# IvanIZ/BenchPush

Measured on AMD Instinct MI355X. Metric: env-steps/sec at N=4096 envs (ship-ice-v0), 1/2/4/8 MI355X, higher is better.
Workload: dtype f64

## Files before the change

benchpush_amd/csrc/bp_capi.hip:

```cpp
#include <hip/hip_runtime.h>

#include <cstdio>
#include <cstdlib>
#include <algorithm>
#include <cstring>
#include <map>
#include <mutex>
#include <string>
#include <vector>

#include <fcntl.h>
#include <sys/file.h>
#include <sys/stat.h>
#include <unistd.h>

#include "bp_host_bd.hpp"
#include "bp_boxdelivery.hpp"
#include "bp_policy.hpp"
#include "bp_render.hpp"
#include "bp_state.hpp"
#include "bp_swath.hpp"
#include "bp_lattice.hpp"
#include "bp_track.hpp"
#include "bp_rrt.hpp"
// ... 52 lines not shown
    std::vector<int> bd_map_of_trial;
    bool timing = false;
    std::vector<hipEvent_t> ev;
    size_t ev_used = 0;
    unsigned long long *cost_ring = nullptr;
    int cost_n = 0;
    int *r_order = nullptr;
    unsigned *r_rgb = nullptr;
    bp_render_prim *r_prims = nullptr;
    int r_nunder = 0, r_nover = 0;
    bool r_table = false;
    unsigned long long scen_hash = 0xCBF29CE484222325ull;
    BpStateLayout st_layout;
    BpStateSeg *st_table = nullptr;
    unsigned long long st_layout_id = 0;
};
#define BP_COST_RING 1024

static int fail(bp_handle *h, int code, const std::string &msg)
{
    if (h) h->err = msg;
    return code;
}
#define HIPCHK(h, call)                                                                                       \
    do {                                                                                                      \
        hipError_t _e = (call);                                                                               \
        if (_e != hipSuccess) return fail((h), BP_EHIP, std::string(#call) + ": " + hipGetErrorString(_e));    \
    } while (0)

struct DevGuard {
    int prev = -1;
// ... 496 lines not shown
    const bool box = h->P.env_kind == BP_ENV_BOX;
    const int cells = box ? h->B.SH * h->B.SW : 0;
    h->st_layout = bp_state_layout(h->D, h->Q, h->nbcap, box, cells);
    const BpStateLayout &L = h->st_layout;
    if (L.nseg >= BP_STATE_MAXSEG || (L.bytes >> 4) >= 0xFFFFFFFFull) return fail(h, BP_EINVAL, "state record layout out of range");
    unsigned long long id = bp_state_structure_id(L, h->P.env_kind, box ? h->bdcfg.task : 0, h->nbcap, cells);
    if (box) id = bp_fnv1a(&h->bdcfg, sizeof(h->bdcfg), id);
    else id = bp_fnv1a(&h->cfg, sizeof(h->cfg), id);
    h->st_layout_id = bp_fnv1a_i64((long long)h->scen_hash, id);
    int rc = dalloc(h, &h->st_table, (size_t)BP_STATE_MAXSEG);
    if (rc) return rc;
    HIPCHK(h, hipMemcpy(h->st_table, L.seg, sizeof(BpStateSeg) * L.nseg, hipMemcpyHostToDevice));
    return BP_OK;
}

static int kind_of(int ctype, int group, int btype) { return ctype | (group << 8) | (btype << 16); }

int bp_load_scenarios(bp_handle *h, int32_t T, int32_t F, int32_t V, const double *verts, const int32_t *counts,
                      const double *centres, const double *starts, const int32_t *nfloes)
{
    if (!h || T <= 0 || F < 0 || V <= 0 || !starts || !nfloes) return BP_EINVAL;
    if (h->loaded) return fail(h, BP_ESTATE, "scenarios already loaded");
    if (h->P.env_kind != BP_ENV_SHIP_ICE) return fail(h, BP_ESTATE, "handle was created for another environment");
    BP_DEVICE(h);
    using namespace bpgeom;
    std::vector<std::vector<Shape>> trials(T);
    for (int t = 0; t < T; t++) {
        std::vector<Shape> &bodies = trials[t];
        Shape ship;
        build_ship(h->cfg.ship_verts, h->cfg.num_ship_verts, starts[3 * t], starts[3 * t + 1], starts[3 * t + 2], ship);
// ... 2 lines not shown
        bodies.push_back(ship);
        if (nfloes[t] > F) return fail(h, BP_EINVAL, "nfloes > F");
        for (int f = 0; f < nfloes[t]; f++) {
            const int n = counts[(size_t)t * F + f];
            if (n < 3) continue;
            if (n > V) return fail(h, BP_EINVAL, "vertex count > V");
            Shape s;
            if (!build_floe(verts + ((size_t)t * F + f) * V * 2, n, centres[((size_t)t * F + f) * 2],
                            centres[((size_t)t * F + f) * 2 + 1], h->cfg.density, h->cfg.poly_radius, s))
                continue;
            s.radius = h->cfg.poly_radius; s.e = h->cfg.elasticity; s.u = h->cfg.friction;
            s.kind = kind_of(2, 0, BODY_DYNAMIC);
            bodies.push_back(s);
        }
    }
    const int rc_up = upload_trials(h, trials);
    return rc_up ? rc_up : state_setup(h);
}

int bp_load_maze(bp_handle *h, int32_t T, int32_t nbox, const double *centres, int32_t nwalls, const double *walls, const double *start)
{
    if (!h || T <= 0 || nbox < 0 || nwalls < 0 || nwalls > 16 || !walls || !start || (nbox > 0 && !centres)) return BP_EINVAL;
    if (h->loaded) return fail(h, BP_ESTATE, "scenarios already loaded");
    if (h->P.env_kind != BP_ENV_MAZE) return fail(h, BP_ESTATE, "handle was created for another environment");
    BP_DEVICE(h);
    using namespace bpgeom;
    const bp_config &cf = h->cfg;
    std::vector<std::vector<Shape>> trials(T);
    for (int t = 0; t < T; t++) {
        std::vector<Shape> &bodies = trials[t];
        for (int k = 0; k <= cf.num_wheels; k++) {
            Shape s;
// ... 34 lines not shown
    {
        std::vector<double> packed(norm.size());
        for (size_t i = 0; i < norm.size(); i++) packed[i] = wall[i] ? -norm[i] : norm[i];
        double *d_pk;
        if ((rc = dalloc(h, &d_pk, packed.size()))) return rc;
        HIPCHK(h, hipMemcpy(d_pk, packed.data(), sizeof(double) * packed.size(), hipMemcpyHostToDevice));
        h->D.maze_obs_map = d_pk;
    }
    double *d_raw;
    if ((rc = dalloc(h, &d_raw, h->goal_raw.size()))) return rc;
    HIPCHK(h, hipMemcpy(d_raw, h->goal_raw.data(), sizeof(double) * h->goal_raw.size(), hipMemcpyHostToDevice));
    h->D.goal_raw = d_raw;
    h->scen_hash = bp_fnv1a(wall.data(), wall.size(), h->scen_hash);
    h->scen_hash = bp_fnv1a(norm.data(), sizeof(double) * norm.size(), h->scen_hash);
    h->scen_hash = bp_fnv1a(h->goal_raw.data(), sizeof(double) * h->goal_raw.size(), h->scen_hash);
    const int rc_up = upload_trials(h, trials);
    return rc_up ? rc_up : state_setup(h);
}

int bp_get_goal_map(bp_handle *h, double *out_host, int32_t *grid_h, int32_t *grid_w)
{
    if (!h) return BP_EINVAL;
    if (h->goal_raw.empty()) return fail(h, BP_ESTATE, "no goal map (not a maze handle or not loaded)");
    if (out_host) memcpy(out_host, h->goal_raw.data(), sizeof(double) * h->goal_raw.size());
    if (grid_h) *grid_h = h->P.grid_h;
    if (grid_w) *grid_w = h->P.grid_w;
    return BP_OK;
}

__device__ __forceinline__ double bp_round2(double x)
{
    const double y = x * 100.0;
// ... 202 lines not shown
        HIPCHK(h, hipGetLastError());
        hipLaunchKernelGGL(k_task_metrics, dim3((E + 255) / 256), dim3(256), 0, st, h->P, h->B, h->D, h->Q, 1, mask, (const unsigned char *)nullptr);
        HIPCHK(h, hipGetLastError());
    }
    if (e1) HIPCHK(h, hipEventRecord(e1, st));
    if (obs) { if (int rc = bd_observe(h, h->B, st, mask, obs)) return rc; }
    if (e2) HIPCHK(h, hipEventRecord(e2, st));
    return BP_OK;
}
static int launch_rigid(bp_handle *h, int mode, const double *actions, const unsigned char *mask, const StepOut &out, hipStream_t st, bool physics, bool raster,
                        hipEvent_t e1, hipEvent_t e2)
{
    unsigned char *obs = out.obs, *term = out.term, *trunc = out.trunc;
    double *reward = out.reward, *info = out.info;
    if (physics) {
        if (mode == MODE_STEP && h->steps_done) {
            hipLaunchKernelGGL(k_make_order, dim3(1), dim3(1024), 0, st, (const unsigned *)h->D.e_cost, h->order_buf, h->num_envs, h->D.sq_thr);
            HIPCHK(h, hipGetLastError());
            h->D.order = h->order_buf;
        }
        if (mode == MODE_STEP) h->steps_done = true;
        if (mode == MODE_STEP && h->pair_mode == 1 && h->D.dbg == nullptr)
            hipLaunchKernelGGL(k_physics_step_pair, dim3((h->num_envs + 1) / 2), dim3(64), 2 * PL_HALF, st, h->P, h->D, actions, reward, term, trunc, info);
        else if (mode == MODE_STEP && h->sched_chunk > 0 && h->D.dbg == nullptr) {
            hipLaunchKernelGGL(k_sched_init, dim3(16), dim3(1024), 0, st, h->P, h->D);
            HIPCHK(h, hipGetLastError());
            if (h->resident_auto && (++h->launches & 63u) == 0) h->device_shared = resident_device_shared(h);
            const bool resident_ok = !(h->resident_auto && h->device_shared);
            if (h->sched_persist && resident_ok) {
                DevParams *Pg = (DevParams *)h->pd_buf;
                DevPtrs *Dg = (DevPtrs *)((char *)h->pd_buf + sizeof(DevParams));
                hipLaunchKernelGGL(k_store_params, dim3(1), dim3(64), 0, st, h->P, h->D, Pg, Dg);
                HIPCHK(h, hipGetLastError());
                if (h->maze8)
                    hipLaunchKernelGGL(k_physics_step_schedl_maze, dim3(h->sched_persist), dim3(64), h->sched_lds, st, Pg, Dg, actions, reward, term, trunc, info);
                else
                    hipLaunchKernelGGL(k_physics_step_schedl, dim3(h->sched_persist), dim3(64), h->sched_lds, st, Pg, Dg, actions, reward, term, trunc, info);
            } else if (h->pair_resident > 0 && h->P.pair_mode == 2 && resident_ok) {
                DevParams *Pg = (DevParams *)h->pd_buf;
                DevPtrs *Dg = (DevPtrs *)((char *)h->pd_buf + sizeof(DevParams));
                hipLaunchKernelGGL(k_store_params, dim3(1), dim3(64), 0, st, h->P, h->D, Pg, Dg);
                HIPCHK(h, hipGetLastError());
                hipLaunchKernelGGL(k_physics_step_schedr, dim3(h->pair_resident), dim3(64), h->sched_lds, st, Pg, Dg, actions, reward, term, trunc, info);
            } else if (h->maze8)
                hipLaunchKernelGGL(k_physics_step_sched_maze, dim3(h->num_envs * h->P.sq_levels), dim3(64), h->sched_lds, st, h->P, h->D, actions, reward, term, trunc, info);
            else if (h->P.pair_mode == 2) {
                if (!h->st_aux) {
                    HIPCHK(h, hipStreamCreateWithFlags(&h->st_aux, hipStreamNonBlocking));
                    HIPCHK(h, hipEventCreateWithFlags(&h->ev_fork, hipEventDisableTiming));
                    HIPCHK(h, hipEventCreateWithFlags(&h->ev_join, hipEventDisableTiming));
                }
                if (h->P.pair_solo > 0) {
                    HIPCHK(h, hipEventRecord(h->ev_fork, st));
                    HIPCHK(h, hipStreamWaitEvent(h->st_aux, h->ev_fork, 0));
                    hipLaunchKernelGGL(k_physics_step_sched, dim3(h->P.pair_solo), dim3(64), h->sched_lds, h->st_aux, h->P, h->D, actions, reward, term, trunc, info);
                    HIPCHK(h, hipGetLastError());
                    HIPCHK(h, hipEventRecord(h->ev_join, h->st_aux));
// ... 38 lines not shown
                    hipLaunchKernelGGL(k_physics_step_sched, dim3(std::min(h->num_envs, SQ_RESCUE)), dim3(64), h->sched_lds, st, PC, h->D, actions, reward, term, trunc, info);
            }
        }
        else if (mode == MODE_STEP && h->damp)
            hipLaunchKernelGGL(k_physics_step_damp, dim3(h->num_envs), dim3(64), h->lds_bytes, st, h->P, h->D, actions, reward, term, trunc, info);
        else if (h->resettle && h->damp)
            hipLaunchKernelGGL(k_physics_reset_damp, dim3(h->num_envs), dim3(64), h->lds_bytes, st, h->P, h->D, mask, info, 0);
        else if (mode == MODE_STEP && h->maze8)
            hipLaunchKernelGGL(k_physics_step_maze, dim3(h->num_envs), dim3(64), h->lds_bytes, st, h->P, h->D, actions, reward, term, trunc, info);
        else if (mode == MODE_STEP)
            hipLaunchKernelGGL(k_physics_step, dim3(h->num_envs), dim3(64), h->lds_bytes, st, h->P, h->D, actions, reward, term, trunc, info);
        else if (h->resettle && h->maze8)
            hipLaunchKernelGGL(k_physics_reset_maze, dim3(h->num_envs), dim3(64), h->lds_bytes, st, h->P, h->D, mask, info, 0);
        else if (h->resettle)
            hipLaunchKernelGGL(k_physics_reset, dim3(h->num_envs), dim3(64), h->lds_bytes, st, h->P, h->D, mask, info, 0);
        else
            hipLaunchKernelGGL(k_reset_copy, dim3(h->num_envs), dim3(256), 0, st, h->P, h->D, mask, info);
        HIPCHK(h, hipGetLastError());
        if (mode == MODE_STEP && h->timing && h->cost_ring && h->cost_n < BP_COST_RING) {
            hipLaunchKernelGGL(k_cost_stats, dim3(1), dim3(1024), 0, st, (const unsigned *)h->D.e_cost, h->num_envs, h->cost_ring, h->cost_n);
            HIPCHK(h, hipGetLastError());
            h->cost_n++;
        }
        if (h->P.env_kind == BP_ENV_SHIP_ICE || h->P.env_kind == BP_ENV_MAZE) {
            hipLaunchKernelGGL(k_episode_metrics, dim3((h->num_envs + 255) / 256), dim3(256), 0, st, h->P, h->D, mode == MODE_STEP ? 0 : 1, mask);
            HIPCHK(h, hipGetLastError());
        }
    }
    if (h->timing) HIPCHK(h, hipEventRecord(e1, st));
    if (raster && obs) {
        if (h->P.env_kind == BP_ENV_MAZE)
            hipLaunchKernelGGL(k_observe_maze, dim3(h->num_envs), dim3(OBS_THREADS), h->obs_lds_bytes, st, h->P, h->D, mask, obs);
        else
            hipLaunchKernelGGL(k_observe, dim3(h->num_envs), dim3(OBS_THREADS_SHIP), h->obs_lds_bytes, st, h->P, h->D, mask, obs);
        HIPCHK(h, hipGetLastError());
    }
    if (h->timing) HIPCHK(h, hipEventRecord(e2, st));
    return BP_OK;
}
static int launch(bp_handle *h, int mode, const double *actions, const unsigned char *mask, const StepOut &out, hipStream_t st, bool physics, bool raster,
                  const AsyncArgs *as = nullptr)
{
    hipEvent_t e0 = nullptr, e1 = nullptr, e2 = nullptr;
    if (h->timing) {
        if (h->ev_used + 3 > h->ev.size()) {
            for (int k = 0; k < 3; k++) { hipEvent_t e; HIPCHK(h, hipEventCreate(&e)); h->ev.push_back(e); }
        }
        e0 = h->ev[h->ev_used]; e1 = h->ev[h->ev_used + 1]; e2 = h->ev[h->ev_used + 2];
        h->ev_used += 3;
// ... 1471 lines not shown
```

benchpush_amd/csrc/bp_kernels.hpp:

```cpp
#pragma once
#include "bp_physics.hpp"

enum { MODE_STEP = 0, MODE_RESET = 1 };

extern __shared__ double2 bp_smem[];

__device__ __forceinline__ double poly_area_seq(const d2 *v, int n)
{
    double d1 = 0.0, d2_ = 0.0;
    for (int i = 0; i < n; i++) {
        const int p = (i - 1 + n) % n;
        d1 += v[i].x * v[p].y;
        d2_ += v[i].y * v[p].x;
    }
    return 0.5 * __builtin_fabs(d1 - d2_);
}
__device__ __forceinline__ d2 poly_centroid_seq(const d2 *v, int n)
{
    const double A = poly_area_seq(v, n);
    double sx = 0.0, sy = 0.0;
    for (int i = 0; i < n; i++) {
        const int p = (i - 1 + n) % n;
        const double u = v[i].x * v[p].y - v[p].x * v[i].y;
        sx += (v[i].x + v[p].x) * u;
// ... 750 lines not shown
    physics_body<MODE_STEP, 0>(P, D, actions, nullptr, reward, terminated, truncated, info, 0);
}
__global__ __launch_bounds__(64, 2) void k_physics_step_pair(const DevParams P, const DevPtrs D, const double *__restrict__ actions,
                                                          double *__restrict__ reward, unsigned char *__restrict__ terminated,
                                                          unsigned char *__restrict__ truncated, double *__restrict__ info)
{
    const int p0 = P.pair_solo ? (int)blockIdx.x : 2 * (int)blockIdx.x, p1 = P.pair_solo ? P.num_envs - 1 - (int)blockIdx.x : p0 + 1;
    const int e0 = D.order != nullptr ? D.order[p0] : p0;
    const int e1 = (p1 < P.num_envs && p1 != p0) ? (D.order != nullptr ? D.order[p1] : p1) : -1;
    PairLimits Q;
    Q.max_keys = Q.max_slots = Q.max_mv = Q.max_act = Q.max_work = 0x7FFFFFFF;
    Q.gc_slots = PP_NSLOT - 12; Q.max_rate = 0x7FFFFFFF;
    int it, score, heavy;
    pair_task<false>(P, D, actions, reward, terminated, truncated, info, e0, e1, Q, it, score, heavy, [](const int) { return false; });
}
__global__ void k_sched_init(const DevParams P, const DevPtrs D)
{
    const int tid = blockIdx.x * blockDim.x + threadIdx.x, nthr = gridDim.x * blockDim.x;
    const int nrows = P.sq_lrpt ? SQ_MAXLEV : P.sq_levels;
    for (int i = tid; i < SQ_NX * nrows * P.sq_cap; i += nthr) {
        const int xk = i / (nrows * P.sq_cap), r = i - xk * (nrows * P.sq_cap);
        D.sq_items[(size_t)xk * SQ_MAXLEV * P.sq_cap + r] = -1;
    }
    for (int i = tid; i < SQ_NX * (SQ_MAXLEV + 2) * 2; i += nthr) D.sq_ctr[i] = 0;
    for (int i = tid; i < P.num_envs; i += nthr) { D.sq_done[i] = 0; D.sq_lev[i] = 0; D.sq_sub[i] = 0; }
}
#define SQ_RESCUE 256
__global__ __launch_bounds__(256) void k_sched_scan(const DevParams P, const DevPtrs D)
{
    __shared__ int cnt;
    if (threadIdx.x == 0) cnt = 0;
    __syncthreads();
    if (sq_ld(sq_finished(D)) < P.num_envs)
// ... 278 lines not shown
        if (pe0 >= 0) {
            const int r = sched_fn_pair<KIND>(Pg, Dg, actions, reward, terminated, truncated, info, pe0, pe1, x, bid < nfirst ? 1 : 0);
            if (r < 0) { __syncthreads(); continue; }
            item = r & 0x3FFFFFF; lev = (int)((unsigned)r >> 26);
        }
        sched_fn_solo<KIND>(Pg, Dg, actions, reward, terminated, truncated, info, item, lev, x);
        __syncthreads();
    }
}
__global__ __launch_bounds__(64, 2) void k_physics_step_schedr(const DevParams *Pg, const DevPtrs *Dg, const double *__restrict__ actions,
                                                            double *__restrict__ reward, unsigned char *__restrict__ terminated,
                                                            unsigned char *__restrict__ truncated, double *__restrict__ info)
{
    sched_resident_pairing<0>(Pg, Dg, actions, reward, terminated, truncated, info);
}
__global__ void k_store_params(const DevParams P, const DevPtrs D, DevParams *Pg, DevPtrs *Dg)
{
    static_assert(sizeof(DevParams) % 4 == 0 && sizeof(DevPtrs) % 4 == 0, "copied as 32-bit words");
    const unsigned *sp = (const unsigned *)&P, *sd = (const unsigned *)&D;
    for (unsigned i = threadIdx.x; i < sizeof(DevParams) / 4; i += blockDim.x) ((unsigned *)Pg)[i] = sp[i];
    for (unsigned i = threadIdx.x; i < sizeof(DevPtrs) / 4; i += blockDim.x) ((unsigned *)Dg)[i] = sd[i];
}
__global__ __launch_bounds__(64, BP_SCHED_WAVES) void k_physics_step_sched(const DevParams P, const DevPtrs D, const double *__restrict__ actions,
                                                           double *__restrict__ reward, unsigned char *__restrict__ terminated,
                                                           unsigned char *__restrict__ truncated, double *__restrict__ info)
{
    sched_body<0, 0>(P, D, actions, reward, terminated, truncated, info);
}
__global__ __launch_bounds__(64, 2) void k_physics_step_schedp(const DevParams P, const DevPtrs D, const double *__restrict__ actions,
                                                            double *__restrict__ reward, unsigned char *__restrict__ terminated,
                                                            unsigned char *__restrict__ truncated, double *__restrict__ info)
// ... 32 lines not shown
                                                           double *__restrict__ info, const int tmpl)
{
    physics_body<MODE_RESET, BP_ENV_MAZE>(P, D, nullptr, mask, nullptr, nullptr, nullptr, tmpl ? nullptr : info, tmpl);
}
__global__ __launch_bounds__(64, 2) void k_bd_settle(const DevParams P, const DevPtrs D, const unsigned char *__restrict__ mask,
                                                  double *__restrict__ info, const int tmpl)
{
    physics_body<MODE_RESET, BP_ENV_BOX>(P, D, nullptr, mask, nullptr, nullptr, nullptr, tmpl ? nullptr : info, tmpl);
}
__global__ __launch_bounds__(64, 2) void k_bd_settle_damp(const DevParams P, const DevPtrs D, const unsigned char *__restrict__ mask,
                                                       double *__restrict__ info, const int tmpl)
{
    physics_body<MODE_RESET, BP_ENV_BOX, false, true>(P, D, nullptr, mask, nullptr, nullptr, nullptr, tmpl ? nullptr : info, tmpl);
}

__global__ __launch_bounds__(1024) void k_make_order(const unsigned *__restrict__ cost, int *__restrict__ order, int n, unsigned *__restrict__ thr)
{
    __shared__ unsigned hist[257];
    __shared__ unsigned smax;
    const int tid = threadIdx.x;
    if (tid < 257) hist[tid] = 0;
    if (tid == 0) smax = 1;
    __syncthreads();
    unsigned mx = 0;
    for (int i = tid; i < n; i += blockDim.x) mx = max(mx, cost[i]);
    atomicMax(&smax, mx);
    __syncthreads();
    const unsigned long long m = smax;
    for (int i = tid; i < n; i += blockDim.x) {
        const unsigned b = 255u - (unsigned)(((unsigned long long)cost[i] * 255ull) / m);
        atomicAdd(&hist[b], 1u);
// ... 1 lines not shown
    __syncthreads();
    if (tid == 0) {
        unsigned acc = 0;
        const unsigned rank = (unsigned)max(1, n / 256);
        int tb = -1;
        for (int b = 0; b < 256; b++) { const unsigned c = hist[b]; hist[b] = acc; acc += c; if (tb < 0 && acc >= rank) tb = b; }
        if (thr != nullptr) thr[0] = (unsigned)((m * (unsigned long long)(255 - max(tb, 0))) / 255ull);
    }
    __syncthreads();
    for (int i = tid; i < n; i += blockDim.x) {
        const unsigned b = 255u - (unsigned)(((unsigned long long)cost[i] * 255ull) / m);
        const unsigned pos = atomicAdd(&hist[b], 1u);
        order[pos] = i;
    }
}


__global__ __launch_bounds__(1024) void k_cost_stats(const unsigned *__restrict__ cost, int n, unsigned long long *__restrict__ ring, int slot)
{
    __shared__ unsigned long long ssum;
    __shared__ unsigned smax;
    if (threadIdx.x == 0) { ssum = 0ull; smax = 0u; }
    __syncthreads();
    unsigned long long s = 0ull;
    unsigned mx = 0u;
    for (int i = threadIdx.x; i < n; i += blockDim.x) { const unsigned c = cost[i]; s += c; mx = max(mx, c); }
    atomicAdd(&ssum, s);
    atomicMax(&smax, mx);
    __syncthreads();
    if (threadIdx.x == 0) { ring[2 * slot] = ssum; ring[2 * slot + 1] = smax; }
}
// ... 231 lines not shown
    while (p < pe) *p++ = flag;
}


#ifdef BP_PROF
#define OPROF(k) { if (tid == 0 && D.prof != nullptr) D.prof[(size_t)env * BP_PROFN + 56 + (k)] = __builtin_amdgcn_s_memtime(); }
#else
#define OPROF(k)
#endif
#define OBS_F_OCC 1u
#define OBS_F_SHIP 2u
#define OBS_F_LINE 4u
#define OBS_F_HEAD 8u

__global__ __launch_bounds__(OBS_THREADS_SHIP, 8) void k_observe(const DevParams P, const DevPtrs D, const unsigned char *__restrict__ mask,
                                                         unsigned char *__restrict__ obs)
{
    const int env = blockIdx.x;
    if (mask != nullptr && mask[env] == 0) return;
    const int tid = threadIdx.x;
    const int nbcap = P.nbcap;
    const size_t eb = (size_t)env * nbcap;
    const int nb = D.e_nb[env];
    const d2 *wv = D.wv + eb * BP_MAXV;
    const int *nv = D.sc_nv + (size_t)D.e_trial[env] * nbcap;
    const int Hg = P.grid_h, Wg = P.grid_w, LH = P.obs_h, LW = P.obs_w;
    const int npix = LH * LW;

    extern __shared__ double2 obs_smem[];
    unsigned char *s_img = (unsigned char *)obs_smem;
    unsigned char *s_edt = s_img + ((npix + 15) & ~15);
    double *s_px = (double *)(s_edt + ((LH + 15) & ~15));
    double *s_py = s_px + OBS_CHUNK * BP_MAXV;
// ... 159 lines not shown
                const long long gj = line.x0 + ax * line.sx, gi = line.y0 + ay * line.sy;
                if (gi >= gi0 && gi <= gi1 && gj >= gj0 && gj <= gj1 && gi >= 0 && gi < Hg && gj >= 0 && gj < Wg) {
                    const int b = ((int)gi - gi0) * LW + ((int)gj - gj0);
                    obs_or_bytes((unsigned *)s_img, b, b, (unsigned char)OBS_F_LINE);
                }
            }
        }
        if (l2 == 0 && hpy >= gi0 && hpy <= gi1 && hpx >= gj0 && hpx <= gj1) {
            const int b = ((int)hpy - gi0) * LW + ((int)hpx - gj0);
            obs_or_bytes((unsigned *)s_img, b, b, (unsigned char)OBS_F_HEAD);
        }
    }
    __syncthreads();
    OPROF(6)
    const size_t plane = (size_t)npix;
    unsigned *o32 = (unsigned *)(obs + (size_t)env * BP_OBS_C * plane);
    const int nwords = npix / 4;
    const int WP = LW / 2, G = OBS_THREADS_SHIP / WP;
    const int g = tid / WP, j = tid - g * WP;
    const int ljlo = max(0, -gj0), ljhi = min(LW - 1, Wg - 1 - gj0);
    if (g < G) {
        const int bs = LW - 4 * j;
        const unsigned mlo = obs_upto(bs);
        const unsigned mA = mlo & obs_upto(ljhi - 4 * j + 1) & ~obs_upto(ljlo - 4 * j);
        const unsigned mB = ~mlo & obs_upto(bs + ljhi + 1) & ~obs_upto(bs + ljlo);
        for (int rp = g; 2 * rp < LH; rp += G) {
            const int w = rp * WP + j;
            const unsigned f = ((const unsigned *)s_img)[w];
            const int giA = gi0 + 2 * rp, giB = giA + 1;
            const unsigned rowA = (giA >= 0 && giA < Hg) ? 0xFFFFFFFFu : 0u, rowB = (giB >= 0 && giB < Hg) ? 0xFFFFFFFFu : 0u;
            const unsigned inb = (rowA & mA) | (rowB & mB);
            const unsigned e2 = ((const unsigned short *)s_edt)[rp];
            const unsigned eA = (e2 & 0xFFu) * 0x01010101u, eB = (e2 >> 8) * 0x01010101u;
            const unsigned e = ((eA & mlo) | (eB & ~mlo)) & inb;
            const unsigned ship = (f >> 1) & 0x01010101u, ln = (f >> 2) & 0x01010101u, hd = (f >> 3) & 0x01010101u;
            o32[w] = inb & (0x7F7F7F7Fu + ship * 0x80u);
            o32[nwords + w] = e | ~inb;
            o32[2 * nwords + w] = inb & ((ln & ~hd) * 127u + hd * 255u);
            o32[3 * nwords + w] = (f & 0x01010101u) * 255u;
        }
    }
    OPROF(7)
}

#define MZ_MAXBOX 64
__global__ __launch_bounds__(OBS_THREADS) void k_observe_maze(const DevParams P, const DevPtrs D, const unsigned char *__restrict__ mask,
                                                              unsigned char *__restrict__ obs)
{
    const int env = blockIdx.x;
    if (mask != nullptr && mask[env] == 0) return;
    const int tid = threadIdx.x;
    const int nbcap = P.nbcap;
    const size_t eb = (size_t)env * nbcap;
    const int nb = D.e_nb[env];
    const size_t tb = (size_t)D.e_trial[env] * nbcap;
    const d2 *wv = D.wv + eb * BP_MAXV;
    const int *nv = D.sc_nv + tb;
    const int *kind = D.sc_kind + tb;
    const int Hg = P.grid_h, Wg = P.grid_w, LH = P.obs_h, LW = P.obs_w;
    const int infl = (LW > LH ? LW : LH) / 2;
    const int IH = LH + infl, IW = LW + infl;
    const int nwords = (IH * IW + 31) / 32;

    extern __shared__ double2 obs_smem[];
// ... 81 lines not shown
            if (gi < 0 || gi >= Hg || gj < 0 || gj >= Wg) continue;
            if (pip_arrays(s_fc, s_fr, s_fcnt, (double)gj, (double)gi)) {
                const int bit = (gi - gi0) * IW + (gj - gj0);
                atomicOr(&s_foot[bit >> 5], 1u << (bit & 31));
            }
        }
    }
    __syncthreads();
    double rs, rc;
    bp_sincos(sa - BP_PI / 2, rs, rc);
    const double ctr = ((double)IH - 1) / 2;
    const double oc0 = rc * ctr + rs * ctr, oc1 = -rs * ctr + rc * ctr;
    const double off0 = ctr - oc0, off1 = ctr - oc1;
    const int half = infl / 2;
    const size_t plane = (size_t)LH * LW;
    unsigned char *o = obs + (size_t)env * BP_OBS_C * plane;
    const int nbits = IH * IW;
    auto sample = [&](const double di, const double dj, unsigned &b0, unsigned &b1, unsigned &b2, unsigned &b3) {
        double c0 = 0.0, c1 = 0.0;
        c0 += di * rc; c0 += dj * rs; c0 += off0;
        c1 += di * -rs; c1 += dj * rc; c1 += off1;
        const bool outside = (c0 < 0 || c0 > IH - 1 || c1 < 0 || c1 > IW - 1);
        const double c0c = outside ? 0.0 : c0, c1c = outside ? 0.0 : c1;
        const double fl0 = __builtin_floor(c0c), fl1 = __builtin_floor(c1c);
        const int s0 = (int)fl0, s1 = (int)fl1;
        const double x0 = c0c - fl0, x1 = c1c - fl1;
        const double w0[2] = {1.0 - x0, x0}, w1[2] = {1.0 - x1, x1};
        double pm[4];
        unsigned wf[4], wb[4];
        bool in[4];
        int sh[4];
// ... 223 lines not shown
```

benchpush_amd/csrc/bp_state.hpp:

```cpp
#pragma once
#include "bp_boxdelivery.hpp"

#define BP_STATE_MAGIC 0x3130534D41504221ull
#define BP_STATE_HDR 32
#define BP_STATE_MAXSEG 64
#define BP_STATE_THREADS 256
enum { BP_SEG_COPY = 0, BP_SEG_OR32 = 1, BP_SEG_HEADER = 2 };

struct BpStateHeader {
    unsigned long long magic, bytes, layout_id, reserved;
};
static_assert(sizeof(BpStateHeader) == BP_STATE_HDR, "record header");

struct BpStateSeg {
    unsigned char *base;
    unsigned long long span;
    unsigned long long off;
    unsigned width;
    unsigned kind;
};
struct BpStateLayout {
    int nseg = 0;
    unsigned long long bytes = 0;
    BpStateSeg seg[BP_STATE_MAXSEG];
// ... 172 lines not shown
            if (MODE == STATE_PACK)
                *(uint4 *)rslot = in == 0 ? make_uint4((unsigned)A.hdr.magic, (unsigned)(A.hdr.magic >> 32), (unsigned)A.hdr.bytes, (unsigned)(A.hdr.bytes >> 32))
                                          : make_uint4((unsigned)A.hdr.layout_id, (unsigned)(A.hdr.layout_id >> 32), 0u, 0u);
            continue;
        }
        const uint4 v = MODE == STATE_UNPACK ? *(const uint4 *)rslot : state_ld(S.base + ea * S.span + in, S.width, n);
        if (MODE == STATE_PACK) { *(uint4 *)rslot = v; continue; }
        unsigned char *const d = S.base + (MODE == STATE_CLONE ? eb : ea) * S.span + in;
        if (S.kind == BP_SEG_OR32) { if (v.x) atomicOr((int *)d, (int)v.x); }
        else state_st(d, S.width, n, v);
    }
}
template <int U> __global__ __launch_bounds__(BP_STATE_THREADS) void k_state_pack(const StateArgs A) { state_body<STATE_PACK, U>(A); }
template <int U> __global__ __launch_bounds__(BP_STATE_THREADS) void k_state_unpack(const StateArgs A) { state_body<STATE_UNPACK, U>(A); }
template <int U> __global__ __launch_bounds__(BP_STATE_THREADS) void k_state_clone(const StateArgs A) { state_body<STATE_CLONE, U>(A); }
```

benchpush_amd/envs/ship_ice.py:

```python
import ctypes as C
import math
import os

import numpy as np
import torch

from .. import _lib
from ..config import DotDict, default_cfg, merge_user_cfg, ship_ice_physics_params
from ..gym_shim import Env, spaces
from ..scenario import generate_ice_field, load_experiment, pack_trials

__all__ = ["BatchedShipIceEnv", "ShipIceEnv", "default_trials"]

_CONC_GEN = {
    0.1: dict(min_r=0.40, max_r=0.58), 0.2: dict(min_r=0.40, max_r=0.58), 0.3: dict(min_r=0.40, max_r=0.58),
    0.4: dict(min_r=0.40, max_r=0.58), 0.5: dict(min_r=0.40, max_r=0.58),
}


def default_trials(concentration, num_trials, base_seed=0, goal_y=9.0):
    kw = _CONC_GEN.get(round(float(concentration), 2), dict(min_r=0.40, max_r=0.58))
    return [generate_ice_field(float(concentration), base_seed + i, goal_y=goal_y, **kw) for i in range(num_trials)]


# ... 126 lines not shown

    def close(self):
        if getattr(self, "h", None):
            self.L.bp_destroy(self.h)
            self.h = None

    def __del__(self):
        try:
            self.close()
        except Exception:
            pass

    def reset(self, mask=None):
        m = None
        if mask is not None:
            m = mask.to(device=self.device, dtype=torch.uint8).contiguous()
        _lib.check(self.L, self.h, self.L.bp_reset(self.h, _ptr(m), _ptr(self.obs), _ptr(self.info), self._stream()), "bp_reset")
        return self.obs, self.info

    def step(self, actions):
        self._actions.copy_(actions.reshape(-1).to(self.device), non_blocking=True)
        _lib.check(self.L, self.h, self.L.bp_step(self.h, _ptr(self._actions), _ptr(self.obs), _ptr(self.reward),
                                                 _ptr(self.terminated), _ptr(self.truncated), _ptr(self.info),
                                                 self._stream()), "bp_step")
        return self.obs, self.reward, self.terminated, self.truncated, self.info

    def step_physics(self, actions):
        self._actions.copy_(actions.reshape(-1).to(self.device), non_blocking=True)
        _lib.check(self.L, self.h, self.L.bp_step_physics(self.h, _ptr(self._actions), _ptr(self.reward), _ptr(self.terminated),
                                                         _ptr(self.truncated), _ptr(self.info), self._stream()), "bp_step_physics")
        return self.reward, self.terminated, self.truncated, self.info

    def observe(self, mask=None):
        m = None if mask is None else mask.to(device=self.device, dtype=torch.uint8).contiguous()
        _lib.check(self.L, self.h, self.L.bp_observe(self.h, _ptr(m), _ptr(self.obs), self._stream()), "bp_observe")
        return self.obs

# ... 456 lines not shown
```

Measured before the change: 299,400.

## Fuse step prologue kernels, add template-based reset with cached observations, skip host copies

Merges k_make_order, k_sched_init and k_store_params into one prologue kernel so each step issues fewer launches. When start positions are not random, the per-trial initial observation is rendered once at load. Auto-reset then copies the cached template state plus that observation with a multi-block copy kernel, instead of re-rendering the observation for reset envs. The Python step and reset paths also pass actions and masks straight through when they already match the expected dtype and device, avoiding a copy. Costs: more device memory for the cached observations, and a per-env ticket counter with atomics to finalize each env reset.

```diff
diff --git a/benchpush_amd/csrc/bp_capi.hip b/benchpush_amd/csrc/bp_capi.hip
--- a/benchpush_amd/csrc/bp_capi.hip
+++ b/benchpush_amd/csrc/bp_capi.hip
@@ -90,7 +90,13 @@
     BpStateLayout st_layout;
     BpStateSeg *st_table = nullptr;
     unsigned long long st_layout_id = 0;
+    unsigned char *tobs = nullptr;
+    BpStateSeg *rs_table = nullptr;
+    int rs_nseg = 0;
+    unsigned rs_nslots = 0;
+    int *rs_ticket = nullptr;
 };
+#define BP_TEMPLATE_OBS_CAP ((size_t)64 << 20)
 #define BP_COST_RING 1024
 
 static int fail(bp_handle *h, int code, const std::string &msg)
@@ -617,6 +623,34 @@
     return BP_OK;
 }
 
+static size_t obs_row_bytes(const bp_handle *h) { return (size_t)BP_OBS_C * h->P.obs_h * h->P.obs_w; }
+
+static int reset_template_setup(bp_handle *h)
+{
+    if (const char *ev = getenv("BP_RESET_TEMPLATE_OBS")) if (atoi(ev) == 0) return BP_OK;
+    if (h->P.random_start) return BP_OK;
+    const int T = h->num_trials;
+    const size_t row = obs_row_bytes(h);
+    if (row % 16 != 0 || (size_t)T * row > BP_TEMPLATE_OBS_CAP) return BP_OK;
+    const BpStateLayout L = bp_reset_layout(h->D, h->nbcap);
+    if (L.nseg >= BP_STATE_MAXSEG || (L.bytes >> 4) + (row >> 4) >= 0xFFFFFFFFull) return BP_OK;
+    int rc;
+    if ((rc = dalloc(h, &h->rs_table, (size_t)BP_STATE_MAXSEG))) return rc;
+    HIPCHK(h, hipMemcpy(h->rs_table, L.seg, sizeof(BpStateSeg) * L.nseg, hipMemcpyHostToDevice));
+    h->rs_nseg = L.nseg; h->rs_nslots = (unsigned)(L.bytes >> 4);
+    if ((rc = dalloc(h, &h->rs_ticket, (size_t)h->num_envs))) return rc;
+    unsigned char *d_tobs;
+    if ((rc = dalloc(h, &d_tobs, (size_t)T * row))) return rc;
+    if (h->P.env_kind == BP_ENV_MAZE)
+        hipLaunchKernelGGL(k_observe_maze, dim3(T), dim3(OBS_THREADS), h->obs_lds_bytes, 0, h->P, h->D, (const unsigned char *)nullptr, d_tobs, h->num_envs);
+    else
+        hipLaunchKernelGGL(k_observe, dim3(T), dim3(OBS_THREADS_SHIP), h->obs_lds_bytes, 0, h->P, h->D, (const unsigned char *)nullptr, d_tobs, h->num_envs);
+    HIPCHK(h, hipGetLastError());
+    HIPCHK(h, hipDeviceSynchronize());
+    h->tobs = d_tobs;
+    return BP_OK;
+}
+
 static int kind_of(int ctype, int group, int btype) { return ctype | (group << 8) | (btype << 16); }
 
 int bp_load_scenarios(bp_handle *h, int32_t T, int32_t F, int32_t V, const double *verts, const int32_t *counts,
@@ -649,8 +683,9 @@
             bodies.push_back(s);
         }
     }
-    const int rc_up = upload_trials(h, trials);
-    return rc_up ? rc_up : state_setup(h);
+    if (int rc_up = upload_trials(h, trials)) return rc_up;
+    if (int rc_t = reset_template_setup(h)) return rc_t;
+    return state_setup(h);
 }
 
 int bp_load_maze(bp_handle *h, int32_t T, int32_t nbox, const double *centres, int32_t nwalls, const double *walls, const double *start)
@@ -715,8 +750,9 @@
     h->scen_hash = bp_fnv1a(wall.data(), wall.size(), h->scen_hash);
     h->scen_hash = bp_fnv1a(norm.data(), sizeof(double) * norm.size(), h->scen_hash);
     h->scen_hash = bp_fnv1a(h->goal_raw.data(), sizeof(double) * h->goal_raw.size(), h->scen_hash);
-    const int rc_up = upload_trials(h, trials);
-    return rc_up ? rc_up : state_setup(h);
+    if (int rc_up = upload_trials(h, trials)) return rc_up;
+    if (int rc_t = reset_template_setup(h)) return rc_t;
+    return state_setup(h);
 }
 
 int bp_get_goal_map(bp_handle *h, double *out_host, int32_t *grid_h, int32_t *grid_w)
@@ -949,7 +985,19 @@
     unsigned char *obs = out.obs, *term = out.term, *trunc = out.trunc;
     double *reward = out.reward, *info = out.info;
     if (physics) {
-        if (mode == MODE_STEP && h->steps_done) {
+        const bool sched_step = mode == MODE_STEP && h->sched_chunk > 0 && h->D.dbg == nullptr && h->pair_mode != 1;
+        DevParams *const Pg = (DevParams *)h->pd_buf;
+        DevPtrs *const Dg = h->pd_buf ? (DevPtrs *)((char *)h->pd_buf + sizeof(DevParams)) : nullptr;
+        bool resident_ok = false;
+        if (sched_step) {
+            if (h->resident_auto && (++h->launches & 63u) == 0) h->device_shared = resident_device_shared(h);
+            resident_ok = !(h->resident_auto && h->device_shared);
+            const bool store = resident_ok && h->pd_buf && (h->sched_persist || (h->pair_resident > 0 && h->P.pair_mode == 2));
+            if (h->steps_done) h->D.order = h->order_buf;
+            hipLaunchKernelGGL(k_step_prologue, dim3(BP_PROLOGUE_BLOCKS), dim3(1024), 0, st, h->P, h->D, h->steps_done ? h->order_buf : (int *)nullptr,
+                               store ? Pg : (DevParams *)nullptr, store ? Dg : (DevPtrs *)nullptr);
+            HIPCHK(h, hipGetLastError());
+        } else if (mode == MODE_STEP && h->steps_done) {
             hipLaunchKernelGGL(k_make_order, dim3(1), dim3(1024), 0, st, (const unsigned *)h->D.e_cost, h->order_buf, h->num_envs, h->D.sq_thr);
             HIPCHK(h, hipGetLastError());
             h->D.order = h->order_buf;
@@ -957,25 +1005,13 @@
         if (mode == MODE_STEP) h->steps_done = true;
         if (mode == MODE_STEP && h->pair_mode == 1 && h->D.dbg == nullptr)
             hipLaunchKernelGGL(k_physics_step_pair, dim3((h->num_envs + 1) / 2), dim3(64), 2 * PL_HALF, st, h->P, h->D, actions, reward, term, trunc, info);
-        else if (mode == MODE_STEP && h->sched_chunk > 0 && h->D.dbg == nullptr) {
-            hipLaunchKernelGGL(k_sched_init, dim3(16), dim3(1024), 0, st, h->P, h->D);
-            HIPCHK(h, hipGetLastError());
-            if (h->resident_auto && (++h->launches & 63u) == 0) h->device_shared = resident_device_shared(h);
-            const bool resident_ok = !(h->resident_auto && h->device_shared);
+        else if (sched_step) {
             if (h->sched_persist && resident_ok) {
-                DevParams *Pg = (DevParams *)h->pd_buf;
-                DevPtrs *Dg = (DevPtrs *)((char *)h->pd_buf + sizeof(DevParams));
-                hipLaunchKernelGGL(k_store_params, dim3(1), dim3(64), 0, st, h->P, h->D, Pg, Dg);
-                HIPCHK(h, hipGetLastError());
                 if (h->maze8)
                     hipLaunchKernelGGL(k_physics_step_schedl_maze, dim3(h->sched_persist), dim3(64), h->sched_lds, st, Pg, Dg, actions, reward, term, trunc, info);
                 else
                     hipLaunchKernelGGL(k_physics_step_schedl, dim3(h->sched_persist), dim3(64), h->sched_lds, st, Pg, Dg, actions, reward, term, trunc, info);
             } else if (h->pair_resident > 0 && h->P.pair_mode == 2 && resident_ok) {
-                DevParams *Pg = (DevParams *)h->pd_buf;
-                DevPtrs *Dg = (DevPtrs *)((char *)h->pd_buf + sizeof(DevParams));
-                hipLaunchKernelGGL(k_store_params, dim3(1), dim3(64), 0, st, h->P, h->D, Pg, Dg);
-                HIPCHK(h, hipGetLastError());
                 hipLaunchKernelGGL(k_physics_step_schedr, dim3(h->pair_resident), dim3(64), h->sched_lds, st, Pg, Dg, actions, reward, term, trunc, info);
             } else if (h->maze8)
                 hipLaunchKernelGGL(k_physics_step_sched_maze, dim3(h->num_envs * h->P.sq_levels), dim3(64), h->sched_lds, st, h->P, h->D, actions, reward, term, trunc, info);
@@ -1044,7 +1080,16 @@
             hipLaunchKernelGGL(k_physics_reset_maze, dim3(h->num_envs), dim3(64), h->lds_bytes, st, h->P, h->D, mask, info, 0);
         else if (h->resettle)
             hipLaunchKernelGGL(k_physics_reset, dim3(h->num_envs), dim3(64), h->lds_bytes, st, h->P, h->D, mask, info, 0);
-        else
+        else if (h->tobs && !(raster && obs && ((uintptr_t)obs & 15u))) {
+            ResetArgs A;
+            A.table = h->rs_table; A.nseg = h->rs_nseg; A.nslots = h->rs_nslots; A.ticket = h->rs_ticket;
+            A.obs16 = (raster && obs) ? (unsigned)(obs_row_bytes(h) >> 4) : 0u;
+            A.tobs = (const uint4 *)h->tobs; A.obs = (uint4 *)obs;
+            const unsigned per_wg = BP_STATE_THREADS * BP_RESET_U;
+            const unsigned pieces = std::min(8u, (A.nslots + A.obs16 + per_wg - 1) / per_wg);
+            hipLaunchKernelGGL(k_reset_template, dim3(h->num_envs, std::max(1u, pieces)), dim3(BP_STATE_THREADS), 0, st, h->P, h->D, A, mask, info);
+            if (A.obs16) obs = nullptr;
+        } else
             hipLaunchKernelGGL(k_reset_copy, dim3(h->num_envs), dim3(256), 0, st, h->P, h->D, mask, info);
         HIPCHK(h, hipGetLastError());
         if (mode == MODE_STEP && h->timing && h->cost_ring && h->cost_n < BP_COST_RING) {
@@ -1060,9 +1105,9 @@
     if (h->timing) HIPCHK(h, hipEventRecord(e1, st));
     if (raster && obs) {
         if (h->P.env_kind == BP_ENV_MAZE)
-            hipLaunchKernelGGL(k_observe_maze, dim3(h->num_envs), dim3(OBS_THREADS), h->obs_lds_bytes, st, h->P, h->D, mask, obs);
+            hipLaunchKernelGGL(k_observe_maze, dim3(h->num_envs), dim3(OBS_THREADS), h->obs_lds_bytes, st, h->P, h->D, mask, obs, 0);
         else
-            hipLaunchKernelGGL(k_observe, dim3(h->num_envs), dim3(OBS_THREADS_SHIP), h->obs_lds_bytes, st, h->P, h->D, mask, obs);
+            hipLaunchKernelGGL(k_observe, dim3(h->num_envs), dim3(OBS_THREADS_SHIP), h->obs_lds_bytes, st, h->P, h->D, mask, obs, 0);
         HIPCHK(h, hipGetLastError());
     }
     if (h->timing) HIPCHK(h, hipEventRecord(e2, st));
diff --git a/benchpush_amd/csrc/bp_kernels.hpp b/benchpush_amd/csrc/bp_kernels.hpp
--- a/benchpush_amd/csrc/bp_kernels.hpp
+++ b/benchpush_amd/csrc/bp_kernels.hpp
@@ -788,9 +788,8 @@
     int it, score, heavy;
     pair_task<false>(P, D, actions, reward, terminated, truncated, info, e0, e1, Q, it, score, heavy, [](const int) { return false; });
 }
-__global__ void k_sched_init(const DevParams P, const DevPtrs D)
-{
-    const int tid = blockIdx.x * blockDim.x + threadIdx.x, nthr = gridDim.x * blockDim.x;
+__device__ __forceinline__ void sched_init_part(const DevParams &P, const DevPtrs &D, const int tid, const int nthr)
+{
     const int nrows = P.sq_lrpt ? SQ_MAXLEV : P.sq_levels;
     for (int i = tid; i < SQ_NX * nrows * P.sq_cap; i += nthr) {
         const int xk = i / (nrows * P.sq_cap), r = i - xk * (nrows * P.sq_cap);
@@ -1099,7 +1098,7 @@
 {
     sched_resident_pairing<0>(Pg, Dg, actions, reward, terminated, truncated, info);
 }
-__global__ void k_store_params(const DevParams P, const DevPtrs D, DevParams *Pg, DevPtrs *Dg)
+__device__ __forceinline__ void store_params_part(const DevParams &P, const DevPtrs &D, DevParams *Pg, DevPtrs *Dg)
 {
     static_assert(sizeof(DevParams) % 4 == 0 && sizeof(DevPtrs) % 4 == 0, "copied as 32-bit words");
     const unsigned *sp = (const unsigned *)&P, *sd = (const unsigned *)&D;
@@ -1162,7 +1161,7 @@
     physics_body<MODE_RESET, BP_ENV_BOX, false, true>(P, D, nullptr, mask, nullptr, nullptr, nullptr, tmpl ? nullptr : info, tmpl);
 }
 
-__global__ __launch_bounds__(1024) void k_make_order(const unsigned *__restrict__ cost, int *__restrict__ order, int n, unsigned *__restrict__ thr)
+__device__ __forceinline__ void make_order_part(const unsigned *__restrict__ cost, int *__restrict__ order, int n, unsigned *__restrict__ thr)
 {
     __shared__ unsigned hist[257];
     __shared__ unsigned smax;
@@ -1194,7 +1193,19 @@
         order[pos] = i;
     }
 }
-
+__global__ __launch_bounds__(1024) void k_make_order(const unsigned *__restrict__ cost, int *__restrict__ order, int n, unsigned *__restrict__ thr)
+{
+    make_order_part(cost, order, n, thr);
+}
+#define BP_PROLOGUE_INIT 16
+#define BP_PROLOGUE_BLOCKS (BP_PROLOGUE_INIT + 2)
+__global__ __launch_bounds__(1024) void k_step_prologue(const DevParams P, const DevPtrs D, int *__restrict__ order, DevParams *Pg, DevPtrs *Dg)
+{
+    const int b = blockIdx.x;
+    if (b == 0) { if (order != nullptr) make_order_part((const unsigned *)D.e_cost, order, P.num_envs, D.sq_thr); }
+    else if (b <= BP_PROLOGUE_INIT) sched_init_part(P, D, (b - 1) * (int)blockDim.x + (int)threadIdx.x, BP_PROLOGUE_INIT * (int)blockDim.x);
+    else if (Pg != nullptr) store_params_part(P, D, Pg, Dg);
+}
 
 __global__ __launch_bounds__(1024) void k_cost_stats(const unsigned *__restrict__ cost, int n, unsigned long long *__restrict__ ring, int slot)
 {
@@ -1456,9 +1467,9 @@
 #define OBS_F_HEAD 8u
 
 __global__ __launch_bounds__(OBS_THREADS_SHIP, 8) void k_observe(const DevParams P, const DevPtrs D, const unsigned char *__restrict__ mask,
-                                                         unsigned char *__restrict__ obs)
-{
-    const int env = blockIdx.x;
+                                                         unsigned char *__restrict__ obs, const int env0)
+{
+    const int env = env0 + blockIdx.x;
     if (mask != nullptr && mask[env] == 0) return;
     const int tid = threadIdx.x;
     const int nbcap = P.nbcap;
@@ -1648,7 +1659,7 @@
     __syncthreads();
     OPROF(6)
     const size_t plane = (size_t)npix;
-    unsigned *o32 = (unsigned *)(obs + (size_t)env * BP_OBS_C * plane);
+    unsigned *o32 = (unsigned *)(obs + (size_t)blockIdx.x * BP_OBS_C * plane);
     const int nwords = npix / 4;
     const int WP = LW / 2, G = OBS_THREADS_SHIP / WP;
     const int g = tid / WP, j = tid - g * WP;
@@ -1679,9 +1690,9 @@
 
 #define MZ_MAXBOX 64
 __global__ __launch_bounds__(OBS_THREADS) void k_observe_maze(const DevParams P, const DevPtrs D, const unsigned char *__restrict__ mask,
-                                                              unsigned char *__restrict__ obs)
-{
-    const int env = blockIdx.x;
+                                                              unsigned char *__restrict__ obs, const int env0)
+{
+    const int env = env0 + blockIdx.x;
     if (mask != nullptr && mask[env] == 0) return;
     const int tid = threadIdx.x;
     const int nbcap = P.nbcap;
@@ -1793,7 +1804,7 @@
     const double off0 = ctr - oc0, off1 = ctr - oc1;
     const int half = infl / 2;
     const size_t plane = (size_t)LH * LW;
-    unsigned char *o = obs + (size_t)env * BP_OBS_C * plane;
+    unsigned char *o = obs + (size_t)blockIdx.x * BP_OBS_C * plane;
     const int nbits = IH * IW;
     auto sample = [&](const double di, const double dj, unsigned &b0, unsigned &b1, unsigned &b2, unsigned &b3) {
         double c0 = 0.0, c1 = 0.0;
diff --git a/benchpush_amd/csrc/bp_state.hpp b/benchpush_amd/csrc/bp_state.hpp
--- a/benchpush_amd/csrc/bp_state.hpp
+++ b/benchpush_amd/csrc/bp_state.hpp
@@ -210,3 +210,94 @@
 template <int U> __global__ __launch_bounds__(BP_STATE_THREADS) void k_state_pack(const StateArgs A) { state_body<STATE_PACK, U>(A); }
 template <int U> __global__ __launch_bounds__(BP_STATE_THREADS) void k_state_unpack(const StateArgs A) { state_body<STATE_UNPACK, U>(A); }
 template <int U> __global__ __launch_bounds__(BP_STATE_THREADS) void k_state_clone(const StateArgs A) { state_body<STATE_CLONE, U>(A); }
+
+#define BP_RESET_U 4
+inline BpStateLayout bp_reset_layout(const DevPtrs &D, int nbcap)
+{
+    BpStateLayout L;
+    const unsigned long long nb = (unsigned long long)nbcap;
+#define BP_SEG_D(arr, elems) bp_state_add(L, #arr, D.arr, sizeof(*D.arr) * (unsigned long long)(elems))
+    BP_SEG_D(pxy, nb); BP_SEG_D(ang, nb); BP_SEG_D(rot, nb); BP_SEG_D(velv, nb); BP_SEG_D(velw, nb); BP_SEG_D(velb, nb);
+    BP_SEG_D(wv, nb * BP_MAXV); BP_SEG_D(wn, nb * BP_MAXV); BP_SEG_D(pv, nb * BP_MAXV);
+    BP_SEG_D(bb, nb); BP_SEG_D(fat, nb);
+    BP_SEG_D(adj, nb * BP_KADJ); BP_SEG_D(hint, nb * BP_KADJ); BP_SEG_D(adjn, nb);
+    BP_SEG_D(a_key, BP_ACAP); BP_SEG_D(a_stamp, BP_ACAP); BP_SEG_D(a_sc, BP_ACAP); BP_SEG_D(a_h0, BP_ACAP); BP_SEG_D(a_h1, BP_ACAP);
+    BP_SEG_D(a_d, BP_ACAP * 14);
+#undef BP_SEG_D
+    return L;
+}
+struct ResetArgs {
+    const BpStateSeg *table;
+    int nseg;
+    unsigned nslots;
+    unsigned obs16;
+    const uint4 *tobs;
+    uint4 *obs;
+    int *ticket;
+};
+__global__ __launch_bounds__(BP_STATE_THREADS) void k_reset_template(const DevParams P, const DevPtrs D, const ResetArgs A, const unsigned char *__restrict__ mask,
+                                                                     double *__restrict__ info)
+{
+    const int env = blockIdx.x;
+    if (mask != nullptr && mask[env] == 0) return;
+    __shared__ BpStateSeg s_seg[BP_STATE_MAXSEG];
+    __shared__ unsigned s_first[BP_STATE_MAXSEG + 1];
+    __shared__ int s_last;
+    const unsigned tid = threadIdx.x;
+    if (tid < (unsigned)A.nseg) { const BpStateSeg s = A.table[tid]; s_seg[tid] = s; s_first[tid] = (unsigned)(s.off >> 4); }
+    if (tid == 0) s_first[A.nseg] = A.nslots;
+    const int episode = D.e_episode[env] + 1;
+    const int trial = (int)(((long long)P.env_offset + env + episode) % P.num_trials);
+    const unsigned long long se = (unsigned long long)(P.num_envs + trial);
+    __syncthreads();
+    const unsigned total = A.nslots + A.obs16, stride = gridDim.y * BP_STATE_THREADS * BP_RESET_U;
+    for (unsigned base = blockIdx.y * BP_STATE_THREADS * BP_RESET_U; base < total; base += stride) {
+        uint4 val[BP_RESET_U];
+        unsigned char *dst[BP_RESET_U];
+        unsigned wd[BP_RESET_U], nn[BP_RESET_U];
+#pragma unroll
+        for (int u = 0; u < BP_RESET_U; u++) {
+            const unsigned slot = base + u * BP_STATE_THREADS + tid;
+            dst[u] = nullptr; wd[u] = 16u; nn[u] = 16u;
+            if (slot >= total) continue;
+            if (slot >= A.nslots) {
+                const unsigned k = slot - A.nslots;
+                val[u] = A.tobs[(size_t)trial * A.obs16 + k];
+                dst[u] = (unsigned char *)(A.obs + (size_t)env * A.obs16 + k);
+                continue;
+            }
+            int lo = 0, hi = A.nseg;
+            while (hi - lo > 1) { const int mid = (lo + hi) >> 1; if (s_first[mid] <= slot) lo = mid; else hi = mid; }
+            const BpStateSeg S = s_seg[lo];
+            const unsigned long long in = (unsigned long long)(slot - s_first[lo]) << 4;
+            if (in >= S.span) continue;
+            wd[u] = S.width; nn[u] = (unsigned)(S.span - in < 16ull ? S.span - in : 16ull);
+            val[u] = state_ld(S.base + se * S.span + in, wd[u], nn[u]);
+            dst[u] = S.base + (unsigned long long)env * S.span + in;
+        }
+#pragma unroll
+        for (int u = 0; u < BP_RESET_U; u++) if (dst[u] != nullptr) state_st(dst[u], wd[u], nn[u], val[u]);
+    }
+    __syncthreads();
+    if (tid == 0) {
+        const int t = atomicAdd(&A.ticket[env], 1);
+        s_last = (t == (int)gridDim.y - 1);
+    }
+    __syncthreads();
+    if (!s_last || tid != 0) return;
+    A.ticket[env] = 0;
+    const size_t s = (size_t)se * P.nbcap;
+    D.e_trial[env] = trial; D.e_episode[env] = episode; D.e_nb[env] = D.e_nb[se];
+    D.e_stamp[env] = D.e_stamp[se]; D.e_currdt[env] = D.e_currdt[se];
+    D.e_total_work[env] = 0.0; D.e_ke[env] = D.e_ke[se]; D.e_imp[env] = D.e_imp[se];
+    D.e_flags[env] = 0; D.e_prevdist[env] = 0.0;
+    for (int q = 0; q < 4; q++) D.e_cnt[env * 4 + q] = D.e_cnt[se * 4 + q];
+    if (D.e_err[se]) atomicOr(&D.e_err[env], D.e_err[se]);
+    if (info) {
+        double *o = info + (size_t)env * BP_INFO_COUNT;
+        for (int q = 0; q < BP_INFO_COUNT; q++) o[q] = 0.0;
+        o[BP_I_X] = D.pxy[s].x; o[BP_I_Y] = D.pxy[s].y; o[BP_I_THETA] = D.ang[s];
+        o[BP_I_KE] = D.e_ke[se]; o[BP_I_IMPULSE] = D.e_imp[se];
+        o[BP_I_NPOST] = (double)D.e_cnt[se * 4 + 0]; o[BP_I_NCONTACT] = (double)D.e_cnt[se * 4 + 1]; o[BP_I_NFIRST] = (double)D.e_cnt[se * 4 + 2];
+    }
+}
diff --git a/benchpush_amd/envs/ship_ice.py b/benchpush_amd/envs/ship_ice.py
--- a/benchpush_amd/envs/ship_ice.py
+++ b/benchpush_amd/envs/ship_ice.py
@@ -164,13 +164,21 @@
     def reset(self, mask=None):
         m = None
         if mask is not None:
-            m = mask.to(device=self.device, dtype=torch.uint8).contiguous()
+            if mask.dtype == torch.bool and mask.device == self.obs.device and mask.is_contiguous():
+                m = mask.view(torch.uint8)
+            else:
+                m = mask.to(device=self.device, dtype=torch.uint8).contiguous()
         _lib.check(self.L, self.h, self.L.bp_reset(self.h, _ptr(m), _ptr(self.obs), _ptr(self.info), self._stream()), "bp_reset")
         return self.obs, self.info
 
     def step(self, actions):
-        self._actions.copy_(actions.reshape(-1).to(self.device), non_blocking=True)
-        _lib.check(self.L, self.h, self.L.bp_step(self.h, _ptr(self._actions), _ptr(self.obs), _ptr(self.reward),
+        if (actions.dtype == torch.float64 and actions.device == self.obs.device and actions.is_contiguous()
+                and actions.numel() == self.num_envs):
+            a = actions
+        else:
+            a = self._actions
+            a.copy_(actions.reshape(-1).to(self.device), non_blocking=True)
+        _lib.check(self.L, self.h, self.L.bp_step(self.h, _ptr(a), _ptr(self.obs), _ptr(self.reward),
                                                  _ptr(self.terminated), _ptr(self.truncated), _ptr(self.info),
                                                  self._stream()), "bp_step")
         return self.obs, self.reward, self.terminated, self.truncated, self.info
```

After: 302,000 (median of 6 runs). Within noise of the previous version (+0.9%).
